# TingweiMeng/PDHG-optimal-control

Measured on AMD Instinct MI355X. Metric: PDHG iterations/sec and achieved HBM GB/s on nt×nx[×ny] grid, 1/2/4/8 MI355X, higher is better.
Workload: dtype f64

## Files before the change

include/pdhg.h:

```cpp
#ifndef PDHG_MI355X_H
#define PDHG_MI355X_H

#ifdef __cplusplus
extern "C" {
#endif

#define PDHG_ABI_VERSION 1

typedef enum pdhg_status {
  PDHG_OK = 0,
  PDHG_ERR_ARG = -1,
  PDHG_ERR_UNSUPPORTED = -2,
  PDHG_ERR_HIP = -3,
  PDHG_ERR_STATE = -4,
  PDHG_ERR_NOMEM = -5
} pdhg_status;

typedef struct pdhg_problem {
  int egno;
  int ndim;
  int bc_x, bc_y;
  int nx, ny;
  int T;
  int precision;
// ... 13 lines not shown
  int inner_last;
  int inner_total;
  double err1;
  double err2;
  double err_inner;
  double rho_min, rho_max;
  int nan_seen;
  int first_nan_iter;
} pdhg_stats;

typedef struct pdhg_ctx pdhg_ctx;

const char* pdhg_last_error(void);
int pdhg_abi_version(void);

int pdhg_device_count(int* count);

int pdhg_create(const pdhg_problem* prob, int device, pdhg_ctx** out);
int pdhg_destroy(pdhg_ctx* ctx);

int pdhg_set_state(pdhg_ctx* ctx, const double* phi, const double* rho, const double* alp);
int pdhg_get_state(pdhg_ctx* ctx, double* phi, double* rho, double* alp);
int pdhg_get_phi_bar(pdhg_ctx* ctx, double* phi_bar);
int pdhg_get_rows(pdhg_ctx* ctx, int row0, int nrows, double* phi, double* phi_bar, double* rho, double* alp);
int pdhg_set_phi_bar(pdhg_ctx* ctx, const double* phi_bar);

int pdhg_init_state(pdhg_ctx* ctx, const double* g);

int pdhg_update_primal(pdhg_ctx* ctx, double tau);

int pdhg_update_dual(pdhg_ctx* ctx, double sigma, double eps, int rho_alp_iters, int* inner_used);

int pdhg_errors(pdhg_ctx* ctx, double* err1, double* err2);

int pdhg_inner_error(pdhg_ctx* ctx, double* err);

int pdhg_iterate(pdhg_ctx* ctx, int n_iters, double tau, double sigma, double eps, int rho_alp_iters,
                 pdhg_stats* out);

int pdhg_set_stop_rules(pdhg_ctx* ctx, int stop_on_converge, int stop_on_nan);

int pdhg_synchronize(pdhg_ctx* ctx);

int pdhg_device_bytes(pdhg_ctx* ctx, unsigned long long* bytes);

int pdhg_path_info(pdhg_ctx* ctx, const char* key, int* value);
// ... 95 lines not shown
```

pdhg-optimal-control_amd/csrc/ctx_impl.hpp:

```cpp
#pragma once

#include <hip/hip_runtime.h>

#include <algorithm>
#include <climits>
#include <cmath>
#include <cstring>
#include <map>
#include <memory>
#include <string>
#include <type_traits>
#include <utility>
#include <vector>

#include "kernels_1d.hpp"
#include "kernels_2d.hpp"
#include "kernels_2d_fast.hpp"
#include "kernels_dual_lds.hpp"
#include "kernels_dual_multi.hpp"
#include "kernels_common.hpp"
#include "kernels_xslab.hpp"
#include "kernels_xt_batch.hpp"
#include "kernels_xt_dma.hpp"
#include "kernels_thomas_chunk.hpp"
// ... 609 lines not shown
          case 512: return launch(k_precond_x_t1_2d<512, 4, 512, double>, g, dim3(512), lds, p, twx);
          default: return fail(PDHG_ERR_UNSUPPORTED, "no fp64 one-row x kernel for nx=%d", p.nx);
        }
      }
      if (pp.f64_xt) {
        if (pp.half_real)
          return launch(k_precond_xt_f64_2d<4096, 512, true>, g, dim3(512),
                        (size_t)(Pad<4096>::LINE + TwLds<4096>::SIZE + 4096 + 128) * sizeof(C), p, twx);
        if (p.nx == 1024)
          return launch(k_precond_xt_f64_2d<1024, 256, false, true>, g, dim3(256),
                        (size_t)(Pad<1024>::LINE + TwLds<1024>::SIZE) * sizeof(C), p, twx);
        if (p.nx == 512)
          return launch(k_precond_xt_f64_2d<512, 128, false, true>, g, dim3(128),
                        (size_t)(Pad<512>::LINE + TwLds<512>::SIZE) * sizeof(C), p, twx);
        if (p.nx == 2048) {
          const size_t bpr = (size_t)(Pad<2048>::LINE + TwLds<2048>::SIZE) * sizeof(C);
          switch (pp.xt64_var) {
            case 1: return launch(k_precond_xt_f64_2d<2048, 256, false, false>, g, dim3(256), bpr + 2048 * sizeof(C), p, twx);
            case 2: return launch(k_precond_xt_f64_2d<2048, 256, false, true>, g, dim3(256), bpr, p, twx);
            case 3: return launch(k_precond_xt_f64_2d<2048, 1024, false, true>, g, dim3(1024), bpr, p, twx);
            default: return launch(k_precond_xt_f64_2d<2048, 512, false, true>, g, dim3(512), bpr, p, twx);
          }
        }
        const size_t lds = (size_t)(Pad<4096>::LINE + TwLds<4096>::SIZE + 4096) * sizeof(C);
        if (p.rspec)
          return launch(k_precond_xt_f64_2d<4096, 512, false, false, true>, g, dim3(512), lds, p, twx);
        return launch(k_precond_xt_f64_2d<4096, 512>, g, dim3(512), lds, p, twx);
      }
    }
    return with_xt_fft([&](auto f) {
      return launch(k_precond_xt_2d<R, decltype(f)>, g, dim3(pp.NT2), pp.lds_xt, p, f, twx);
    });
  }

  int launch_update_2d(const KP<R>& p, int& upd_rows) {
    ProfScope ps(this, "update");
    const dim3 gf(pp.g_fast_upd);
    upd_rows = pp.g_fast_upd;
    if constexpr (sizeof(R) == 8) {
      if (pp.res64) {
        if (pb.ny == 2048 && pp.upd_t1 > 0) {
          const size_t lds = pp.lds_res64 + (size_t)48 * sizeof(C);
          if (pp.upd_t1 == 2) return launch(k_invy_update_fast_2d<2048, 4, 256, 2, double, true>, gf, dim3(256), lds, p, twy);
          return launch(k_invy_update_fast_2d<2048, 4, 256, 4, double, true>, gf, dim3(256), lds, p, twy);
        }
        if (pb.ny == 4096) return launch(k_invy_update_fast_2d<4096, 4, 512, 4, double>, gf, dim3(512), pp.lds_upd64, p, twy);
// ... 816 lines not shown

  int set_phi_bar(const double* pbar) {
    const size_t n = (size_t)(pb.T + 1) * plane();
    if constexpr (sizeof(P) == 8) {
      H2D(phibar_dev(), pbar, n * sizeof(P));
      return PDHG_OK;
    }
    std::vector<R> buf(n);
    for (size_t i = 0; i < n; ++i) buf[i] = (R)pbar[i];
    H2D(kp.phibar, buf.data(), n * sizeof(R));
    return PDHG_OK;
  }

  int get_phi_bar(double* pbar) {
    HIP_TRY(hipStreamSynchronize(stream));
    const size_t n = (size_t)(pb.T + 1) * plane();
    if constexpr (kMixed) {
      HIP_TRY(hipMemcpy(pbar, px.phibar, n * sizeof(P), hipMemcpyDeviceToHost));
      return PDHG_OK;
    }
    std::vector<R> buf(n);
    HIP_TRY(hipMemcpy(buf.data(), kp.phibar, n * sizeof(R), hipMemcpyDeviceToHost));
    for (size_t i = 0; i < n; ++i) pbar[i] = (double)buf[i];
    return PDHG_OK;
  }

  int get_state(double* phi, double* rho, double* alp) {
    HIP_TRY(hipStreamSynchronize(stream));
    Ctrl h;
    int rc;
    if ((rc = read_ctrl(h))) return rc;
    const int cur = h.cur;
    const size_t npl = plane();
    const int T = pb.T;
    const size_t nphi = (size_t)(T + 1) * npl;
    std::unique_ptr<R[]> buf(new R[nphi]);
    const size_t n = (size_t)T * npl;
    auto plane_out = [&](double* dst, const auto* src, size_t cnt) -> int {
      using E = std::remove_cv_t<std::remove_pointer_t<decltype(src)>>;
      if constexpr (sizeof(E) == 8) {
        HIP_TRY(hipMemcpy(dst, src, cnt * sizeof(E), hipMemcpyDeviceToHost));
      } else {
        HIP_TRY(hipMemcpy(buf.get(), src, cnt * sizeof(E), hipMemcpyDeviceToHost));
        for (size_t i = 0; i < cnt; ++i) dst[i] = (double)buf[i];
      }
      return PDHG_OK;
// ... 368 lines not shown
```

pdhg-optimal-control_amd/csrc/fft_lds.hpp:

```cpp
#pragma once
#include "common.hpp"

namespace pdhg {

struct FFTPlan {
  int n;
  int npass;
  int pow2;
  int radix[kMaxPass];
};

__device__ constexpr double kC16[16] = {1.0, 0.92387953251128674, 0.70710678118654752, 0.38268343236508977,
                                        0.0, -0.38268343236508977, -0.70710678118654752, -0.92387953251128674,
                                        -1.0, -0.92387953251128674, -0.70710678118654752, -0.38268343236508977,
                                        0.0, 0.38268343236508977, 0.70710678118654752, 0.92387953251128674};
__device__ constexpr double kS16[16] = {0.0, 0.38268343236508977, 0.70710678118654752, 0.92387953251128674,
                                        1.0, 0.92387953251128674, 0.70710678118654752, 0.38268343236508977,
                                        0.0, -0.38268343236508977, -0.70710678118654752, -0.92387953251128674,
                                        -1.0, -0.92387953251128674, -0.70710678118654752, -0.38268343236508977};

template <typename C>
__device__ __forceinline__ void dft2(C& a, C& b) {
  const C t = a;
  a = cadd(t, b);
// ... 327 lines not shown
  lds_sync();
#pragma unroll
  for (int q = 0; q < PER; ++q) {
    if (base[q] >= 0) {
      dft_any<C, R>(v[q]);
      C* d = a + base[q];
#pragma unroll
      for (int r = 0; r < R; ++r) d[(LS == 1) ? r : r * (LS + LS / 16)] = v[q][r];
    }
  }
  lds_sync();
}

template <typename C, int N, int NL, int NT, int LS, bool REG, int LINE = Pad<N>::LINE, int GLS = (1 << 30)>
__device__ __forceinline__ void inplace_passes(C* a, const C* __restrict__ tw, const C* twl) {
  if constexpr (LS < N) {
    constexpr int rem = N / LS;
    constexpr int R = (rem >= 16) ? 16 : rem;
    inplace_pass<C, N, NL, NT, LS, R, REG, LINE, GLS>(a, tw, twl);
    inplace_passes<C, N, NL, NT, LS * R, REG, LINE, GLS>(a, tw, twl);
  }
}

template <typename C, int N, int NL, int NT, int LINE = Pad<N>::LINE>
__device__ __forceinline__ void lds_fft_inplace(C* a, const C* __restrict__ tw) {
  inplace_passes<C, N, NL, NT, 1, false, LINE>(a, tw, nullptr);
}

template <typename C, int N, int NL, int NT, int LINE = Pad<N>::LINE>
__device__ __forceinline__ void lds_fft_inplace_tl(C* a, const C* twl) {
  inplace_passes<C, N, NL, NT, 1, true, LINE>(a, nullptr, twl);
}

template <typename C, int N, int NL, int NT, int LINE = Pad<N>::LINE>
__device__ __forceinline__ void lds_fft_inplace_tl16(C* a, const C* twl, const C* __restrict__ tw) {
  inplace_passes<C, N, NL, NT, 1, true, LINE, 256>(a, tw, twl);
}


template <typename C, int N>
__device__ __forceinline__ void fill_twlds(C* twl, const C* __restrict__ tw, int tw_stride = 1,
                                           int cnt = TwLds<N>::SIZE) {
  for (int i = threadIdx.x; i < cnt; i += blockDim.x) {
    const int LS = i >= 816 ? 4096 : i >= 48 ? 256 : 16;
    const int e = i - twlds_off(LS);
    const int k = e / 3, m = e - 3 * k;
// ... 184 lines not shown
```

pdhg-optimal-control_amd/csrc/kernels_xt_f64.hpp:

```cpp
#pragma once
#include "kernels_2d_fast.hpp"

namespace pdhg {

__device__ __forceinline__ __amdgpu_buffer_rsrc_t row_rsrc(const double* base, int bytes) {
  return __builtin_amdgcn_make_buffer_rsrc(const_cast<double*>(base), 0, bytes, 0x00020000);
}
__device__ __forceinline__ double2 buf_ld2(__amdgpu_buffer_rsrc_t r, int voff, int soff) {
  return __builtin_bit_cast(double2, __builtin_amdgcn_raw_buffer_load_b128(r, voff, soff, 0));
}
__device__ __forceinline__ void buf_st2(__amdgpu_buffer_rsrc_t r, int voff, int soff, double2 v) {
  __builtin_amdgcn_raw_buffer_store_b128(__builtin_bit_cast(u32x4_t, v), r, voff, soff, 0);
}

__device__ __forceinline__ double eth_of(double dd) {
  return 1.0 / (1.0 + 0.5 * dd + sqrt(dd * (1.0 + 0.25 * dd)));
}
__device__ __forceinline__ double theta_of(double dd) {
  const double dl = 0.5 * dd;
  return fmax(log1p(dl + sqrt(dl * (dl + 2.0))), 1e-300);
}


template <int N, int NT, bool HR = false, bool BPR = false, bool TC = false>
__global__ void __launch_bounds__(NT) k_precond_xt_f64_2d(KP<double> p, const double2* __restrict__ twx) {
  using C = double2;
  constexpr int IT = N / NT;
  constexpr int LINE = Pad<N>::LINE;
  constexpr int M = 2 * N;
  static_assert(N % NT == 0 && N <= 4096 && IT <= 32, "one padded complex line and its twiddle seeds in LDS");
  if (p.ctrl->done) return;
  extern __shared__ __align__(16) unsigned char smem_raw[];
  C* A = reinterpret_cast<C*>(smem_raw);
  C* twl = A + LINE;
  C* bp = twl + TwLds<N>::SIZE;
  C* rsw = bp + (BPR ? 0 : N);
  static_assert(!(BPR && HR), "half-real blocks keep b' in LDS");
  static_assert(!TC || (!HR && !BPR && NT % 4 == 0), "task-order input: column pairs, 4-row tasks");
  fill_twlds<C, N>(twl, twx, HR ? 2 : 1);
  if constexpr (HR) {
    static_assert(N == 4096, "split-twiddle tables sized for 2N = 8192");
    for (int i = threadIdx.x; i < 128; i += blockDim.x) rsw[i] = twx[i < 64 ? i : 64 * (i - 64)];
  }
  const int T = p.T, tid = threadIdx.x;
  const int b = ((TC && !(p.dbg & 4096)) ? xcd_remap(blockIdx.x, gridDim.x) : (int)blockIdx.x) + p.b0;
  double* wb = p.work + (size_t)b * M;
  const size_t kstride = (size_t)p.nb * M;
  const double inv_ae = 1.0 / (double)p.ae;
  const double ly0 = p.lamy[HR ? b : 2 * b], ly1 = p.lamy[HR ? b : 2 * b + 1];
  auto kx_of = [&](int i) { return tid + i * NT; };
  auto dd_of = [&](int i) {
    const double lx0 = p.lamx[kx_of(i)], lx1 = HR ? (double)p.lamx[kx_of(i) + N] : lx0;
    return make_double2(((double)p.C - lx0 - ly0) * inv_ae, ((double)p.C - lx1 - ly1) * inv_ae);
  };
  auto unpack2 = [&](int i, double& h0, double& h1) {
    if constexpr (HR) {
      const int k = kx_of(i);
      realsplit_padded<C, double>(A, N, k, cmul(rsw[k & 63], rsw[64 + (k >> 6)]), h0, h1);
    } else {
      hartley_padded<C, double>(A, N, kx_of(i), h0, h1);
    }
  };
  auto stage2 = [&](int i, C x) {
    if constexpr (HR) {
      double* Af = reinterpret_cast<double*>(A);
      const int f0 = kx_of(i), f1 = kx_of(i) + N;
      Af[2 * pix(f0 >> 1) + (f0 & 1)] = x.x;
// ... 30 lines not shown
#pragma unroll
    for (int i = 0; i < IT; ++i) pf[i] = buf_ld2(r, voff, ioff(i));
  };
  const int ny_t = p.nb * 2;
  auto ldrow_in = [&](int kk) {
    if constexpr (TC) {
      const auto r = row_rsrc(p.rspec + (size_t)kk * kstride + (size_t)8 * b, (int)(kstride * sizeof(double)) - 64 * b);
      const int vin = 32 * ny_t * (tid >> 2) + 16 * (tid & 3);
#pragma unroll
      for (int i = 0; i < IT; ++i) pf[i] = buf_ld2(r, vin, 8 * ny_t * NT * i);
    } else {
      ldrow(kk);
    }
  };
  const int j0 = p.j0;
  const bool slab = p.slab != 0;
  if (p.xt_phase != 2) {
#pragma unroll
    for (int i = 0; i < IT; ++i) {
      c1[i] = dd_of(i);
      c2[i] = slab ? make_double2(h_entry(c1[i].x, j0), h_entry(c1[i].y, j0)) : make_double2(1.0, 1.0);
      bp_st(i, make_double2(0.0, 0.0));
    }
    ldrow_in(0);
    for (int k = 0; k < T; ++k) {
      const int kg = j0 + k;
      const bool nrow = k == T - 1 && p.last_slab;
#pragma unroll
      for (int i = 0; i < IT; ++i) A[pix(kx_of(i))] = pf[i];
      if (k + 1 < T) ldrow_in(k + 1);
      lds_sync();
      lds_fft_inplace_tl<C, N, 1, NT>(A, twl);
#pragma unroll
      for (int i = 0; i < IT; ++i)
        if (kg == max(kf[i], j0) && !nrow)
          c1[i] = make_double2(eth_of(c1[i].x), eth_of(c1[i].y));
      const auto dst = rowr(k);
#pragma unroll
      for (int i = 0; i < IT; ++i) {
        double ha, hb;
        unpack2(i, ha, hb);
        const C b0 = bp_ld(i);
        const double r0 = ha * inv_ae + b0.x, r1 = hb * inv_ae + b0.y;
        C bn;
        const int kfj = max(kf[i], j0);
        const bool fast = kg > kfj || (kg == kfj && !nrow);
        if (!nrow) {
          if (fast) {
            bn = make_double2(r0 * c1[i].x, r1 * c1[i].y);
          } else {
            const double s0 = c1[i].x + c2[i].x, s1 = c1[i].y + c2[i].y;
            const double g0 = 1.0 / (1.0 + s0), g1 = 1.0 / (1.0 + s1);
            bn = make_double2(r0 * g0, r1 * g1);
            c2[i] = make_double2(s0 * g0, s1 * g1);
          }
          buf_st2(dst, voff, ioff(i), bn);
        } else {
          if (fast) bn = make_double2(r0 * c1[i].x / (1.0 - c1[i].x), r1 * c1[i].y / (1.0 - c1[i].y));
          else bn = make_double2(r0 / (c1[i].x + c2[i].x), r1 / (c1[i].y + c2[i].y));
          if (slab) buf_st2(dst, voff, ioff(i), bn);
        }
        bp_st(i, bn);
      }
      lds_sync();
    }
  }
  if (p.xt_phase == 1) return;
  const int ks = slab ? T - 1 : T - 2;
#pragma unroll
  for (int i = 0; i < IT; ++i) {
    const C dd = dd_of(i);
    c1[i] = make_double2(theta_of(dd.x), theta_of(dd.y));
    if (j0 + ks >= kf[i]) {
      c2[i] = make_double2(exp(-c1[i].x), exp(-c1[i].y));
    } else {
      c2[i] = make_double2(expm1(-2.0 * c1[i].x * (j0 + ks + 2)), expm1(-2.0 * c1[i].y * (j0 + ks + 2)));
    }
    if (slab) bp_st(i, p.carry_y ? reinterpret_cast<const C*>(p.carry_y + (size_t)b * M)[kx_of(i)]
                                 : make_double2(0.0, 0.0));
  }
  if (ks >= 0) ldrow(ks);
  for (int k = T - 1; k >= 0; --k) {
    const int kg = j0 + k;
#pragma unroll
    for (int i = 0; i < IT; ++i)
      if (kg + 1 == kf[i] && k < ks)
        c2[i] = make_double2(expm1(-2.0 * c1[i].x * (kg + 2)), expm1(-2.0 * c1[i].y * (kg + 2)));
#pragma unroll
    for (int i = 0; i < IT; ++i) {
      C x = bp_ld(i);
      if (k <= ks) {
        double g0, g1;
        if (kg >= kf[i]) {
          g0 = c2[i].x;
          g1 = c2[i].y;
        } else {
          const double t0 = c1[i].x, t1 = c1[i].y;
          const double e0 = expm1(-2.0 * t0 * (kg + 1)), e1 = expm1(-2.0 * t1 * (kg + 1));
          g0 = t0 > 1e-150 ? exp(-t0) * e0 / c2[i].x : (double)(kg + 1) / (double)(kg + 2);
          g1 = t1 > 1e-150 ? exp(-t1) * e1 / c2[i].y : (double)(kg + 1) / (double)(kg + 2);
          c2[i] = make_double2(e0, e1);
        }
        x = make_double2(pf[i].x + g0 * x.x, pf[i].y + g1 * x.y);
        bp_st(i, x);
      }
      stage2(i, x);
// ... 22 lines not shown
```

pdhg-optimal-control_amd/csrc/path_plan.hpp:

```cpp
#pragma once

#include <cstdio>
#include <string>

#include "../../include/pdhg.h"
#include "fft_lds.hpp"
#include "kernels_dual_multi.hpp"
#include "kernels_fs16.hpp"
#include "tuning.hpp"

namespace pdhg {

constexpr size_t kLdsBytes = 160 * 1024;
constexpr int kMultiSub = 5;
constexpr int kMixedUpdPF = 4;
constexpr int kFoldRows = 64;

inline FFTPlan make_plan(int n, bool& ok) {
  FFTPlan pl{};
  pl.n = n;
  pl.pow2 = (n > 0) && ((n & (n - 1)) == 0);
  int m = n, np = 0;
  ok = true;
  auto push = [&](int r) {
// ... 50 lines not shown
  bool k1_outer = true;
  bool fold_fin = false;
  bool spec_ok = false;
  bool fin_merge = true;
  bool fuse_res = false;
  bool fast_rows = false;
  bool res64 = false;
  bool ip_rows = false;
  bool upd8192 = false;
  bool tc_spec = false;
  bool to_c4 = false;
  int res_threads = 0, upd_threads = 0;
  int res64_nt2048 = 512;
  int upd_t1 = 0;
  bool t1_xt = true;
  bool fast_xt = false;
  int fast_xt_code = 0;
  bool xt_dma = false, xt_pair = false;
  int xt_rpre = 0;
  bool t1_xt64 = false;
  bool t1_g16 = false;
  bool f64_xt = false;
  int xt64_var = 0;
  bool glb_line = false;
  bool fourstep = false;
  bool fs_wide = true;
  bool fs16 = false;
  int f16_group = 16;
  bool thomas_chunk = false;
  bool report_tile = false;
  int report_wgs = 1024;
};

inline int plan_paths(const pdhg_problem& pb, int S, const Decomp& dc, const Tuning& tn, PathPlan& pl,
                      std::string& err) {
  auto fail = [&err](int code, const char* fmt, auto... args) {
    if constexpr (sizeof...(args) == 0) {
      err = fmt;
    } else {
      char buf[512];
      snprintf(buf, sizeof(buf), fmt, args...);
      err = buf;
    }
    return code;
  };
  pl = PathPlan{};
// ... 8 lines not shown
  pl.n_dead = (pb.ndim == 2 && pb.egno == 3) ? 2 : 0;
  const bool two_sets = pl.two_sets = pb.rho_alp_iters > 1;
  bool ok1 = true, ok2 = true;
  pl.plx = make_plan(nxg, ok1);
  if (is2d) pl.ply = make_plan(ny, ok2);
  if (!ok1 || !ok2) return fail(PDHG_ERR_UNSUPPORTED, "FFT plan too deep for nx=%d ny=%d", nxg, ny);

  if (is2d) {
    const size_t cap = (S == 4) ? 8192 : 4096;
    int B = 16;
    while (B > 2 && (size_t)nxg * B > cap) B >>= 1;
    int nyp = 2;
    while (nyp < ny) nyp <<= 1;
    if (B > nyp) B = nyp;
    const bool xt64_on = tn.xt64.value_or(1) != 0;
    const bool f64_small = S == 8 && pb.bc_x == 0 && (slab ? dc.Tg : T) > 1 && (nxg == 1024 || nxg == 512) &&
                           ny % 2 == 0 && xt64_on;
    if (f64_small) B = 2;
    pl.half_real = nxg == 8192 && pb.bc_x == 0 && (S == 4 || !xslab);
    if (pl.half_real) B = 1;
    pl.f64_xt = S == 8 && pb.bc_x == 0 &&
                (((nxg == 4096 || nxg == 2048) && B == 2) || (nxg == 8192 && pl.half_real) || f64_small) && xt64_on;
    pl.xt64_var = tn.xt64_var;
    pl.t1_xt64 = S == 8 && T == 1 && pb.bc_x == 0 && !pl.half_real && !slab && pl.plx.pow2 &&
                 nxg >= 512 && nxg <= 4096 && nxg * (B / 2) == (nxg == 4096 ? 4096 : 2048);
    pl.res64_nt2048 = tn.res64_nt2048.value_or(T == 1 ? 256 : 512);
    pl.upd_t1 = T == 1 ? tn.upd_t1.value_or(2) : 0;
    if (!pl.half_real && !pl.f64_xt && (size_t)nxg * B > cap)
      return fail(PDHG_ERR_UNSUPPORTED, "nx=%d too large for the x-transform slab (max %zu in this precision)", nxg,
                  cap / 2);
    pl.B = B;
    while ((1 << pl.lB) < B) ++pl.lB;
    pl.nb = (ny + B - 1) / B;
    pl.lds_res = 2 * (size_t)ny * csz;
    const int nmodes = nxg * B;
    pl.lds_xt = (size_t)5 * nmodes * S;
    pl.ip_rows = S == 8 && ny == 8192 && pl.lds_res > kLdsBytes && !xslab;
    if (pl.ip_rows) pl.lds_res = (size_t)Pad<8192>::LINE * csz;
    pl.upd8192 = pl.ip_rows && pl.half_real && nx % 2 == 0 && tn.upd8192.value_or(1) != 0;
    if (pl.upd8192) pl.g_fast_upd = std::min((nx / 2) * T, 2048);
    if (pl.lds_res > kLdsBytes) return fail(PDHG_ERR_UNSUPPORTED, "ny=%d exceeds the LDS row transform", ny);
    {
      const int wg = (int)std::max<size_t>(1, kLdsBytes / std::max<size_t>(pl.lds_res, 1));
      pl.nt_row = std::min(1024, 256 * std::max(1, 4 / wg));
    }
    pl.NT2 = std::min(512, ((nmodes + 63) / 64) * 64);
// ... 166 lines not shown
  else if (k == "dual64") *value = (S == 8 && pl.fast_dual) ? 1 : 0;
  else if (k == "fast_dual") *value = pl.fast_dual ? pl.dual_rx : -1;
  else if (k == "dual_ypl") *value = pl.fast_dual && pl.dual_rx ? pl.dual_ypl : 0;
  else if (k == "res64_nt") *value = pl.res64 ? (pb.ny == 2048 ? pl.res64_nt2048 : 512) : 0;
  else if (k == "upd_t1") *value = (pl.res64 && pb.ny == 2048) ? pl.upd_t1 : 0;
  else if (k == "t1_g16") *value = (pl.t1_g16 && (pb.nx == 2048 || pb.nx == 4096)) ? 1 : 0;
  else if (k == "dual_one") *value = pl.dual_one ? 1 : 0;
  else if (k == "fast_xt") *value = pl.fast_xt_code;
  else if (k == "half_real") *value = pl.half_real ? 1 : 0;
  else if (k == "fourstep") *value = pl.fourstep ? 1 : 0;
  else if (k == "glb_line") *value = pl.glb_line ? 1 : 0;
  else if (k == "ip_rows") *value = pl.ip_rows ? 1 : 0;
  else if (k == "upd8192") *value = pl.upd8192 ? 1 : 0;
  else if (k == "tc_spec") *value = pl.tc_spec ? 1 : 0;
  else if (k == "to_c4") *value = pl.to_c4 ? 1 : 0;
  else if (k == "thomas_chunk") *value = pl.thomas_chunk ? 1 : 0;
  else if (k == "fs_wide") *value = (pl.fourstep && pl.fs_wide && !pl.fs16) ? 1 : 0;
  else if (k == "fs16") *value = pl.fs16 ? 1 : 0;
  else if (k == "rows_rw") *value = pl.fast_rows ? pl.RWf : 0;
  else if (k == "row_threads") *value = pl.nt_row;
  else if (k == "res_threads") *value = pl.res_threads;
  else if (k == "upd_threads") *value = pl.upd_threads;
  else if (k == "f64_xt") *value = pl.f64_xt ? 1 : 0;
  else if (k == "t1_xt64") *value = (pl.t1_xt64 && pl.t1_xt) ? 1 : 0;
  else if (k == "report_tile") *value = pl.report_tile ? 1 : 0;
  else if (k == "report_wgs") *value = pl.report_tile ? pl.report_wgs : 0;
  else return false;
  return true;
}

}
```

pdhg-optimal-control_amd/csrc/pdhg_api.hip:

```cpp
#include <hip/hip_runtime.h>

#include <cstdarg>
#include <cstdio>
#include <memory>
#include <string>

#include "../../include/pdhg.h"

namespace {

thread_local std::string g_err;

int fail(int code, const char* fmt, ...) {
  char buf[1024];
  va_list ap;
  va_start(ap, fmt);
  vsnprintf(buf, sizeof(buf), fmt, ap);
  va_end(ap);
  g_err = buf;
  return code;
}

#define HIP_TRY(expr)                                                                           \
  do {                                                                                          \
// ... 158 lines not shown
  if (rc) return rc;
  *out = reinterpret_cast<pdhg_ctx*>(box.release());
  return PDHG_OK;
}

int pdhg_destroy(pdhg_ctx* ctx) {
  if (!ctx) return PDHG_OK;
  CtxBox* b = ctx_box(ctx);
  if (!b) return fail(PDHG_ERR_ARG, "foreign context handle");
  b->magic = 0;
  delete b;
  return PDHG_OK;
}

int pdhg_set_state(pdhg_ctx* ctx, const double* phi, const double* rho, const double* alp) {
  return dispatch(ctx, [&](auto& im) { return im.set_state(phi, rho, alp); });
}
int pdhg_get_state(pdhg_ctx* ctx, double* phi, double* rho, double* alp) {
  return dispatch(ctx, [&](auto& im) { return im.get_state(phi, rho, alp); });
}
int pdhg_get_phi_bar(pdhg_ctx* ctx, double* phi_bar) {
  if (!phi_bar) return fail(PDHG_ERR_ARG, "null phi_bar");
  return dispatch(ctx, [&](auto& im) { return im.get_phi_bar(phi_bar); });
}
int pdhg_set_phi_bar(pdhg_ctx* ctx, const double* phi_bar) {
  if (!phi_bar) return fail(PDHG_ERR_ARG, "null phi_bar");
  return dispatch(ctx, [&](auto& im) { return im.set_phi_bar(phi_bar); });
}
int pdhg_get_rows(pdhg_ctx* ctx, int row0, int nrows, double* phi, double* phi_bar, double* rho, double* alp) {
  return dispatch(ctx, [&](auto& im) { return im.get_rows(row0, nrows, phi, phi_bar, rho, alp); });
}
int pdhg_init_state(pdhg_ctx* ctx, const double* g) {
  if (!g) return fail(PDHG_ERR_ARG, "null g");
  return dispatch(ctx, [&](auto& im) { return im.init_state(g); });
}
int pdhg_update_primal(pdhg_ctx* ctx, double tau) {
  return dispatch(ctx, [&](auto& im) { return im.update_primal(tau); });
}
int pdhg_update_dual(pdhg_ctx* ctx, double sigma, double eps, int rho_alp_iters, int* inner_used) {
  if (rho_alp_iters < 1) return fail(PDHG_ERR_ARG, "rho_alp_iters must be >= 1");
  return dispatch(ctx, [&](auto& im) { return im.update_dual(sigma, eps, rho_alp_iters, inner_used); });
}
int pdhg_errors(pdhg_ctx* ctx, double* err1, double* err2) {
  return dispatch(ctx, [&](auto& im) { return im.errors(err1, err2); });
}
int pdhg_inner_error(pdhg_ctx* ctx, double* err) {
// ... 373 lines not shown
```

pdhg-optimal-control_amd/csrc/tuning.hpp:

```cpp
#pragma once

#include <algorithm>
#include <cstdlib>
#include <cstring>
#include <optional>

namespace pdhg {

using EnvInt = std::optional<int>;

inline EnvInt env_int(const char* name) {
  const char* e = getenv(name);
  return e ? EnvInt(atoi(e)) : EnvInt();
}
inline int env_int(const char* name, int dflt) { return env_int(name).value_or(dflt); }
inline bool env_flag(const char* name, bool dflt) { return env_int(name, dflt ? 1 : 0) != 0; }

struct Tuning {
  int alloc_mode = 0;

  EnvInt xt64;
  int xt64_var = 0;
  bool t1_xt = true;
  bool t1_g16 = true;
  int short_t_xt = 16;
  EnvInt xt_ws;
  EnvInt xt_batch;
  int xt_rpre = 0;
  bool xt_pair = false;
  EnvInt xt_dma;
  EnvInt xt_dma_hr;

  EnvInt upd_t1;
  EnvInt res64_nt2048;
  EnvInt upd8192;
  int rows_var = 0;
  int half_nt = 3;
  int res64_nt = 512;
  int upd_pf = 4;
  EnvInt tile_j;
  EnvInt res64;
  EnvInt tc_spec;
  EnvInt fuse_res;
  EnvInt c4_to;

// ... 11 lines not shown
  EnvInt fs16;
  int f16_group = 16;
  EnvInt fuse_res1d;
  int fr1d_chunks = 8;
  EnvInt thomas_chunk;

  bool k1_outer = true;
  bool fold_fin = false;
  int g_outer = 2048;
  int head_xrun = 4;
  EnvInt dual_multi;
  EnvInt dual_head;
  EnvInt spec;
  bool fin_merge = true;

  EnvInt report_tile;
  int report_wgs = 1024;

  static Tuning from_env() {
    Tuning t;
    if (const char* e = getenv("PDHG_ALLOC")) t.alloc_mode = !strcmp(e, "contig") ? 1 : !strcmp(e, "none") ? -1 : 0;
    t.xt64 = env_int("PDHG_XT64");
    t.xt64_var = env_int("PDHG_XT64_VAR", t.xt64_var);
    t.t1_xt = env_flag("PDHG_T1_XT", t.t1_xt);
    t.t1_g16 = env_flag("PDHG_T1_G16", t.t1_g16);
    t.short_t_xt = env_int("PDHG_SHORT_T_XT", t.short_t_xt);
    t.xt_ws = env_int("PDHG_XT_WS");
    t.xt_batch = env_int("PDHG_XT_BATCH");
    t.xt_rpre = env_int("PDHG_XT_RPRE", t.xt_rpre);
    t.xt_pair = env_flag("PDHG_XT_PAIR", t.xt_pair);
    t.xt_dma = env_int("PDHG_XT_DMA");
    t.xt_dma_hr = env_int("PDHG_XT_DMA_HR");
    t.upd_t1 = env_int("PDHG_UPD_T1");
    if ((t.res64_nt2048 = env_int("PDHG_RES64_NT2048"))) t.res64_nt2048 = *t.res64_nt2048 == 256 ? 256 : 512;
    t.upd8192 = env_int("PDHG_UPD8192");
    t.rows_var = env_int("PDHG_ROWS_VAR", t.rows_var);
    t.half_nt = env_int("PDHG_HALF_NT", t.half_nt);
    t.res64_nt = env_int("PDHG_RES64_NT", t.res64_nt) == 1024 ? 1024 : 512;
    t.upd_pf = env_int("PDHG_UPD_PF", t.upd_pf);
    t.tile_j = env_int("PDHG_TILE_J");
    t.res64 = env_int("PDHG_RES64");
    t.tc_spec = env_int("PDHG_TC_SPEC");
    t.fuse_res = env_int("PDHG_FUSE_RES");
    t.c4_to = env_int("PDHG_C4_TO");
    t.short_t_dual = env_int("PDHG_SHORT_T", t.short_t_dual);
    t.dual64 = env_int("PDHG_DUAL64");
// ... 62 lines not shown
```

pdhg-optimal-control_amd/pdhg_amd/_native.py:

```python
import ctypes
import os

import numpy as np

_HERE = os.path.dirname(os.path.abspath(__file__))
LIB_PATH = os.path.join(_HERE, "libpdhg.so")

PDHG_OK = 0
PDHG_ERR_ARG = -1
PDHG_ERR_UNSUPPORTED = -2
PDHG_ERR_HIP = -3
PDHG_ERR_STATE = -4
PDHG_ERR_NOMEM = -5

EXPORTS = (
    "pdhg_last_error", "pdhg_abi_version", "pdhg_device_count", "pdhg_create", "pdhg_destroy",
    "pdhg_set_state", "pdhg_get_state", "pdhg_get_phi_bar", "pdhg_set_phi_bar", "pdhg_get_rows", "pdhg_init_state",
    "pdhg_update_primal", "pdhg_update_dual", "pdhg_errors", "pdhg_inner_error", "pdhg_iterate", "pdhg_set_stop_rules", "pdhg_synchronize",
    "pdhg_device_bytes", "pdhg_path_info", "pdhg_plan_info", "pdhg_profile_enable", "pdhg_profile_query", "pdhg_algorithmic_bytes",
    "pdhg_trajectories",
    "pdhg_report_state", "pdhg_report_rows",
    "pdhg_create_slab", "pdhg_set_stream", "pdhg_slab_plane_size", "pdhg_slab_begin", "pdhg_slab_carry_gain",
    "pdhg_slab_residual", "pdhg_slab_forward", "pdhg_slab_fixup", "pdhg_slab_long_modes", "pdhg_slab_fixup_nb", "pdhg_slab_backward", "pdhg_slab_primal_finalize", "pdhg_slab_dual",
    "pdhg_slab_dual_finalize", "pdhg_slab_outer", "pdhg_slab_outer_finalize", "pdhg_slab_plane_out",
    "pdhg_slab_plane_in", "pdhg_slab_status", "pdhg_slab_part_modes", "pdhg_slab_forward_part",
    "pdhg_slab_carry_out_part", "pdhg_slab_fixup_nb_part", "pdhg_slab_backward_part", "pdhg_slab_update",
    "pdhg_create_xslab", "pdhg_xslab_layout", "pdhg_xslab_sizes", "pdhg_xslab_halo_out", "pdhg_xslab_halo_in",
    "pdhg_xslab_residual", "pdhg_xslab_wire", "pdhg_xslab_precond", "pdhg_xslab_update",
    "pdhg_create_multi", "pdhg_multi_destroy", "pdhg_multi_set_state", "pdhg_multi_get_state",
    "pdhg_multi_iterate", "pdhg_multi_set_stop_rules", "pdhg_multi_synchronize", "pdhg_multi_info",
    "pdhg_multi_profile", "pdhg_multi_phase_ms", "pdhg_multi_init_state", "pdhg_build_id",
)


class PDHGError(RuntimeError):
    def __init__(self, code, msg):
        super().__init__("pdhg status {}: {}".format(code, msg))
        self.code = code


# ... 51 lines not shown

def load():
    global _lib
    if _lib is not None:
        return _lib
    if not os.path.exists(LIB_PATH):
        raise ImportError("libpdhg.so not built at {} — run __graft_entry__.build()".format(LIB_PATH))
    try:
        import torch
    except ImportError:
        pass
    lib = ctypes.CDLL(LIB_PATH)
    P = ctypes.c_void_p
    dp = ctypes.POINTER(ctypes.c_double)
    sig = {
        "pdhg_last_error": ([], ctypes.c_char_p),
        "pdhg_abi_version": ([], ctypes.c_int),
        "pdhg_device_count": ([ctypes.POINTER(ctypes.c_int)], ctypes.c_int),
        "pdhg_create": ([ctypes.POINTER(pdhg_problem), ctypes.c_int, ctypes.POINTER(P)], ctypes.c_int),
        "pdhg_destroy": ([P], ctypes.c_int),
        "pdhg_set_state": ([P, dp, dp, dp], ctypes.c_int),
        "pdhg_get_state": ([P, dp, dp, dp], ctypes.c_int),
        "pdhg_get_phi_bar": ([P, dp], ctypes.c_int),
        "pdhg_set_phi_bar": ([P, dp], ctypes.c_int),
        "pdhg_get_rows": ([P, ctypes.c_int, ctypes.c_int, dp, dp, dp, dp], ctypes.c_int),
        "pdhg_init_state": ([P, dp], ctypes.c_int),
        "pdhg_update_primal": ([P, ctypes.c_double], ctypes.c_int),
        "pdhg_update_dual": ([P, ctypes.c_double, ctypes.c_double, ctypes.c_int, ctypes.POINTER(ctypes.c_int)],
                             ctypes.c_int),
        "pdhg_errors": ([P, dp, dp], ctypes.c_int),
        "pdhg_inner_error": ([P, dp], ctypes.c_int),
        "pdhg_iterate": ([P, ctypes.c_int, ctypes.c_double, ctypes.c_double, ctypes.c_double, ctypes.c_int,
                          ctypes.POINTER(pdhg_stats)], ctypes.c_int),
        "pdhg_set_stop_rules": ([P, ctypes.c_int, ctypes.c_int], ctypes.c_int),
        "pdhg_synchronize": ([P], ctypes.c_int),
        "pdhg_device_bytes": ([P, ctypes.POINTER(ctypes.c_ulonglong)], ctypes.c_int),
        "pdhg_path_info": ([P, ctypes.c_char_p, ctypes.POINTER(ctypes.c_int)], ctypes.c_int),
        "pdhg_plan_info": ([ctypes.POINTER(pdhg_problem), ctypes.c_char_p, ctypes.POINTER(ctypes.c_int)], ctypes.c_int),
        "pdhg_profile_enable": ([P, ctypes.c_int], ctypes.c_int),
        "pdhg_profile_query": ([P, ctypes.c_char_p, dp, ctypes.POINTER(ctypes.c_int)], ctypes.c_int),
        "pdhg_algorithmic_bytes": ([P, ctypes.c_int, ctypes.c_char_p, dp], ctypes.c_int),
        "pdhg_trajectories": ([P, ctypes.POINTER(pdhg_traj_opts), dp, dp, dp, dp, dp], ctypes.c_int),
        "pdhg_report_state": ([P, ctypes.POINTER(pdhg_report)], ctypes.c_int),
        "pdhg_report_rows": ([P, ctypes.c_int, ctypes.c_int, dp, dp], ctypes.c_int),
        "pdhg_create_slab": ([ctypes.POINTER(pdhg_problem), ctypes.c_int, ctypes.c_int, ctypes.c_int,
                              ctypes.POINTER(P)], ctypes.c_int),
# ... 84 lines not shown
```

pdhg-optimal-control_amd/pdhg_amd/context.py:

```python
import ctypes

import numpy as np

from . import _native as N


def traj_arguments(ndim, T, x_init, method, x_period, y_period=None, center=(False, False), noise=None,
                   record=("x", "alp"), seed=0, sample_offset=0):
    if method not in N.TRAJ_METHODS:
        raise ValueError("method must be 'linear' or 'nearest', not {!r}".format(method))
    record = (record,) if isinstance(record, str) else tuple(record or ())
    if set(record) - {"x", "alp"}:
        raise ValueError("record takes 'x' and / or 'alp', not {!r}".format(record))
    x0 = np.ascontiguousarray(x_init, dtype=np.float64)
    want = "[n_sample]" if ndim == 1 else "[n_sample, 2]"
    if x0.ndim != ndim or (ndim == 2 and x0.shape[1] != 2) or x0.shape[0] < 1:
        raise ValueError("x_init must be {} with n_sample >= 1, not {}".format(want, x0.shape))
    n = x0.shape[0]
    if ndim == 2 and y_period is None:
        raise ValueError("y_period is required in 2-D")
    if not (x_period > 0) or (ndim == 2 and not (y_period > 0)):
        raise ValueError("periods must be > 0")
    if len(tuple(center)) != 2:
        raise ValueError("center is a pair (center_x, center_y)")
# ... 94 lines not shown
                len(alp) == len(r[2]) and all(a is b for a, b in zip(alp, r[2])))

    def get_state(self, phi=True, rho=True, alp=True):
        phi = np.empty((self.T + 1,) + self._space) if phi else None
        rho = np.empty((self.T,) + self._space) if rho else None
        alp = np.empty((self.n_alp, self.T) + self._space + (self.n_ctrl,)) if alp else None
        N.check(self._lib.pdhg_get_state(self._h, N.dptr(phi), N.dptr(rho), N.dptr(alp)))
        return phi, rho, (None if alp is None else tuple(alp[i] for i in range(self.n_alp)))

    def get_rows(self, row0, nrows, phi=True, phi_bar=False, rho=True, alp=True):
        sp = self._space
        f = lambda on: np.empty((nrows,) + sp) if on else None
        a = np.empty((self.n_alp, nrows) + sp + (self.n_ctrl,)) if alp else None
        ph, pb, rh = f(phi), f(phi_bar), f(rho)
        N.check(self._lib.pdhg_get_rows(self._h, int(row0), int(nrows), N.dptr(ph), N.dptr(pb), N.dptr(rh),
                                        N.dptr(a)))
        return ph, pb, rh, (None if a is None else tuple(a[i] for i in range(self.n_alp)))

    def get_phi_bar(self):
        pb = np.empty((self.T + 1,) + self._space)
        N.check(self._lib.pdhg_get_phi_bar(self._h, N.dptr(pb)))
        return pb

    def set_phi_bar(self, phi_bar):
        self._version += 1
        pb = np.ascontiguousarray(phi_bar, dtype=np.float64).reshape((self.T + 1,) + self._space)
        N.check(self._lib.pdhg_set_phi_bar(self._h, N.dptr(pb)))

    def init_state(self, g):
        g = np.ascontiguousarray(g, dtype=np.float64).reshape(self._space)
        self._version += 1
        N.check(self._lib.pdhg_init_state(self._h, N.dptr(g)))

    def trajectories(self, x_init, method, x_period, y_period=None, center=(False, False), noise=None, seed=0,
                     record=("x", "alp"), sample_offset=0):
        o, x0, noise, rec_x, rec_a = traj_arguments(self.ndim, self.T, x_init, method, x_period, y_period, center,
                                                    noise, record, seed, sample_offset)
        n = x0.shape[0]
        tail = () if self.ndim == 1 else (2,)
        x_final = np.empty((n,) + tail)
        traj_x = np.empty((self.T + 1, n) + tail) if rec_x else None
        traj_alp = np.empty((self.T, n, self.n_ctrl)) if rec_a else None
        N.check(self._lib.pdhg_trajectories(self._h, ctypes.byref(o), N.dptr(x0), N.dptr(noise), N.dptr(x_final),
                                            N.dptr(traj_x), N.dptr(traj_alp)))
        return traj_alp, traj_x, x_final

# ... 69 lines not shown
```

Baseline: 8.520.

## Stage f64 xt preconditioner rows into LDS with async global-load-to-LDS DMA

For the nx=4096, column-pair f64 xt preconditioner path, adds a DMA variant that prefetches the next time row straight into an LDS staging buffer with global_load_lds. The first FFT pass then reads out-of-place from that buffer with hand-written ds_read_b128 batches, and the b' stores are moved after the FFT with a counted vmcnt wait. It also enables the b'-in-registers (BPR) variant by default for this configuration. The aim is to overlap the HBM row loads with the LDS FFT and free registers, at the cost of more static LDS, inline asm fragility and fixed waitcnt encodings. A debug accessor for the work buffer is added as well.

```diff
diff --git a/include/pdhg.h b/include/pdhg.h
--- a/include/pdhg.h
+++ b/include/pdhg.h
@@ -59,6 +59,7 @@
 int pdhg_set_state(pdhg_ctx* ctx, const double* phi, const double* rho, const double* alp);
 int pdhg_get_state(pdhg_ctx* ctx, double* phi, double* rho, double* alp);
 int pdhg_get_phi_bar(pdhg_ctx* ctx, double* phi_bar);
+int pdhg_get_work(pdhg_ctx* ctx, double* out, long long count);
 int pdhg_get_rows(pdhg_ctx* ctx, int row0, int nrows, double* phi, double* phi_bar, double* rho, double* alp);
 int pdhg_set_phi_bar(pdhg_ctx* ctx, const double* phi_bar);
 
diff --git a/pdhg-optimal-control_amd/csrc/ctx_impl.hpp b/pdhg-optimal-control_amd/csrc/ctx_impl.hpp
--- a/pdhg-optimal-control_amd/csrc/ctx_impl.hpp
+++ b/pdhg-optimal-control_amd/csrc/ctx_impl.hpp
@@ -655,6 +655,15 @@
             default: return launch(k_precond_xt_f64_2d<2048, 512, false, true>, g, dim3(512), bpr, p, twx);
           }
         }
+        if (pp.xt64_dma) {
+          if (p.rspec) return launch(k_precond_xt_f64_2d<4096, 512, false, true, true, true>, g, dim3(512), 0, p, twx);
+          return launch(k_precond_xt_f64_2d<4096, 512, false, true, false, true>, g, dim3(512), 0, p, twx);
+        }
+        if (pp.xt64_bpr) {
+          const size_t ldsr = (size_t)(Pad<4096>::LINE + TwLds<4096>::SIZE) * sizeof(C);
+          if (p.rspec) return launch(k_precond_xt_f64_2d<4096, 512, false, true, true>, g, dim3(512), ldsr, p, twx);
+          return launch(k_precond_xt_f64_2d<4096, 512, false, true>, g, dim3(512), ldsr, p, twx);
+        }
         const size_t lds = (size_t)(Pad<4096>::LINE + TwLds<4096>::SIZE + 4096) * sizeof(C);
         if (p.rspec)
           return launch(k_precond_xt_f64_2d<4096, 512, false, false, true>, g, dim3(512), lds, p, twx);
@@ -1517,6 +1526,16 @@
     std::vector<R> buf(n);
     HIP_TRY(hipMemcpy(buf.data(), kp.phibar, n * sizeof(R), hipMemcpyDeviceToHost));
     for (size_t i = 0; i < n; ++i) pbar[i] = (double)buf[i];
+    return PDHG_OK;
+  }
+
+  int get_work(double* out, size_t count) {
+    HIP_TRY(hipStreamSynchronize(stream));
+    const size_t nwork = pb.ndim == 2 ? (size_t)pb.T * kp.nb * pb.nx * kp.B : (size_t)pb.T * pb.nx;
+    if (count > nwork) return fail(PDHG_ERR_ARG, "work buffer holds %zu elements", nwork);
+    std::vector<R> buf(count);
+    HIP_TRY(hipMemcpy(buf.data(), kp.work, count * sizeof(R), hipMemcpyDeviceToHost));
+    for (size_t i = 0; i < count; ++i) out[i] = (double)buf[i];
     return PDHG_OK;
   }
 
diff --git a/pdhg-optimal-control_amd/csrc/fft_lds.hpp b/pdhg-optimal-control_amd/csrc/fft_lds.hpp
--- a/pdhg-optimal-control_amd/csrc/fft_lds.hpp
+++ b/pdhg-optimal-control_amd/csrc/fft_lds.hpp
@@ -373,6 +373,26 @@
   }
 }
 
+template <typename C, int N, int NT, class RD>
+__device__ __forceinline__ void first_pass_oop(C* __restrict__ a, RD&& read16) {
+  constexpr int nR = N / 16;
+  static_assert(nR % 16 == 0 && nR <= NT, "padded schedule, one butterfly per thread");
+  const int j = threadIdx.x;
+  C v[16];
+  int base = -1;
+  if (j < nR) {
+    read16(j, v);
+    base = pix(j * 16);
+  }
+  asm volatile("" : "+v"(base)::"memory");
+  if (base >= 0) {
+    dft_any<C, 16>(v);
+    C* d = a + base;
+#pragma unroll
+    for (int r = 0; r < 16; ++r) d[r] = v[r];
+  }
+}
+
 template <typename C, int N, int NL, int NT, int LINE = Pad<N>::LINE>
 __device__ __forceinline__ void lds_fft_inplace(C* a, const C* __restrict__ tw) {
   inplace_passes<C, N, NL, NT, 1, false, LINE>(a, tw, nullptr);
diff --git a/pdhg-optimal-control_amd/csrc/kernels_xt_f64.hpp b/pdhg-optimal-control_amd/csrc/kernels_xt_f64.hpp
--- a/pdhg-optimal-control_amd/csrc/kernels_xt_f64.hpp
+++ b/pdhg-optimal-control_amd/csrc/kernels_xt_f64.hpp
@@ -1,5 +1,6 @@
 #pragma once
 #include "kernels_2d_fast.hpp"
+#include "kernels_xt_dma.hpp"
 
 namespace pdhg {
 
@@ -11,6 +12,24 @@
 }
 __device__ __forceinline__ void buf_st2(__amdgpu_buffer_rsrc_t r, int voff, int soff, double2 v) {
   __builtin_amdgcn_raw_buffer_store_b128(__builtin_bit_cast(u32x4_t, v), r, voff, soff, 0);
+}
+
+__device__ __forceinline__ void s_read16(unsigned a, double2 (&v)[16]) {
+  typedef double d2v __attribute__((ext_vector_type(2)));
+  d2v w[16];
+  asm volatile(
+      "ds_read_b128 %0, %16\n\tds_read_b128 %1, %16 offset:4096\n\tds_read_b128 %2, %16 offset:8192\n\t"
+      "ds_read_b128 %3, %16 offset:12288\n\tds_read_b128 %4, %16 offset:16384\n\tds_read_b128 %5, %16 offset:20480\n\t"
+      "ds_read_b128 %6, %16 offset:24576\n\tds_read_b128 %7, %16 offset:28672\n\tds_read_b128 %8, %16 offset:32768\n\t"
+      "ds_read_b128 %9, %16 offset:36864\n\tds_read_b128 %10, %16 offset:40960\n\tds_read_b128 %11, %16 offset:45056\n\t"
+      "ds_read_b128 %12, %16 offset:49152\n\tds_read_b128 %13, %16 offset:53248\n\t"
+      "ds_read_b128 %14, %16 offset:57344\n\tds_read_b128 %15, %16 offset:61440\n\ts_waitcnt lgkmcnt(0)"
+      : "=&v"(w[0]), "=&v"(w[1]), "=&v"(w[2]), "=&v"(w[3]), "=&v"(w[4]), "=&v"(w[5]), "=&v"(w[6]), "=&v"(w[7]),
+        "=&v"(w[8]), "=&v"(w[9]), "=&v"(w[10]), "=&v"(w[11]), "=&v"(w[12]), "=&v"(w[13]), "=&v"(w[14]), "=&v"(w[15])
+      : "v"(a)
+      : "memory");
+#pragma unroll
+  for (int r = 0; r < 16; ++r) v[r] = make_double2(w[r].x, w[r].y);
 }
 
 __device__ __forceinline__ double eth_of(double dd) {
@@ -22,27 +41,39 @@
 }
 
 
-template <int N, int NT, bool HR = false, bool BPR = false, bool TC = false>
+template <int N, int NT, bool HR = false, bool BPR = false, bool TC = false, bool DMA = false>
 __global__ void __launch_bounds__(NT) k_precond_xt_f64_2d(KP<double> p, const double2* __restrict__ twx) {
   using C = double2;
   constexpr int IT = N / NT;
   constexpr int LINE = Pad<N>::LINE;
   constexpr int M = 2 * N;
   static_assert(N % NT == 0 && N <= 4096 && IT <= 32, "one padded complex line and its twiddle seeds in LDS");
+  static_assert(!DMA || (BPR && !HR && N == 4096 && NT == 512), "DMA staging: the nx = 4096 column-pair form");
   if (p.ctrl->done) return;
   extern __shared__ __align__(16) unsigned char smem_raw[];
-  C* A = reinterpret_cast<C*>(smem_raw);
-  C* twl = A + LINE;
+  C *A, *twl, *S = nullptr;
+  if constexpr (DMA) {
+    __shared__ __align__(16) C A_s[LINE];
+    __shared__ __align__(16) C S_s[N];
+    __shared__ __align__(16) C twl_s[TwLds<N>::SIZE];
+    A = A_s;
+    S = S_s;
+    twl = twl_s;
+  } else {
+    A = reinterpret_cast<C*>(smem_raw);
+    twl = A + LINE;
+  }
   C* bp = twl + TwLds<N>::SIZE;
   C* rsw = bp + (BPR ? 0 : N);
   static_assert(!(BPR && HR), "half-real blocks keep b' in LDS");
-  static_assert(!TC || (!HR && !BPR && NT % 4 == 0), "task-order input: column pairs, 4-row tasks");
+  static_assert(!TC || (!HR && NT % 4 == 0), "task-order input: column pairs, 4-row tasks");
   fill_twlds<C, N>(twl, twx, HR ? 2 : 1);
   if constexpr (HR) {
     static_assert(N == 4096, "split-twiddle tables sized for 2N = 8192");
     for (int i = threadIdx.x; i < 128; i += blockDim.x) rsw[i] = twx[i < 64 ? i : 64 * (i - 64)];
   }
-  const int T = p.T, tid = threadIdx.x;
+  const int T = p.T;
+  int tid = threadIdx.x;
   const int b = ((TC && !(p.dbg & 4096)) ? xcd_remap(blockIdx.x, gridDim.x) : (int)blockIdx.x) + p.b0;
   double* wb = p.work + (size_t)b * M;
   const size_t kstride = (size_t)p.nb * M;
@@ -119,15 +150,40 @@
       c2[i] = slab ? make_double2(h_entry(c1[i].x, j0), h_entry(c1[i].y, j0)) : make_double2(1.0, 1.0);
       bp_st(i, make_double2(0.0, 0.0));
     }
-    ldrow_in(0);
+    const int wave = __builtin_amdgcn_readfirstlane(tid >> 6);
+    auto issue_row = [&](auto kk) {
+      const char* src = TC ? reinterpret_cast<const char*>(p.rspec + (size_t)kk * kstride + (size_t)8 * b) +
+                                 (32 * ny_t * (tid >> 2) + 16 * (tid & 3))
+                           : reinterpret_cast<const char*>(wb + (size_t)kk * kstride) + voff;
+#pragma unroll
+      for (int i = 0; i < IT; ++i)
+        __builtin_amdgcn_global_load_lds(
+            reinterpret_cast<const u32x4_t*>(src + (TC ? (size_t)8 * ny_t * NT * i : (size_t)ioff(i))),
+            (__attribute__((address_space(3))) void*)(S + i * NT + wave * 64), 16, 0, 0);
+    };
+    if constexpr (DMA) {
+      issue_row(0);
+      __builtin_amdgcn_s_waitcnt(0x0F70);
+      lds_sync();
+    } else {
+      ldrow_in(0);
+    }
     for (int k = 0; k < T; ++k) {
       const int kg = j0 + k;
       const bool nrow = k == T - 1 && p.last_slab;
-#pragma unroll
-      for (int i = 0; i < IT; ++i) A[pix(kx_of(i))] = pf[i];
-      if (k + 1 < T) ldrow_in(k + 1);
-      lds_sync();
-      lds_fft_inplace_tl<C, N, 1, NT>(A, twl);
+      if constexpr (DMA) {
+        if (!(p.dbg & 8192))
+          first_pass_oop<C, N, NT>(A, [&](int j, C(&v)[16]) { s_read16(lds_addr(S + j), v); });
+        lds_sync();
+        if (k + 1 < T) issue_row(k + 1);
+        inplace_passes<C, N, 1, NT, 16, true>(A, nullptr, twl);
+      } else {
+#pragma unroll
+        for (int i = 0; i < IT; ++i) A[pix(kx_of(i))] = pf[i];
+        if (k + 1 < T) ldrow_in(k + 1);
+        lds_sync();
+        lds_fft_inplace_tl<C, N, 1, NT>(A, twl);
+      }
 #pragma unroll
       for (int i = 0; i < IT; ++i)
         if (kg == max(kf[i], j0) && !nrow)
@@ -151,13 +207,27 @@
             bn = make_double2(r0 * g0, r1 * g1);
             c2[i] = make_double2(s0 * g0, s1 * g1);
           }
-          buf_st2(dst, voff, ioff(i), bn);
+          if constexpr (!DMA) buf_st2(dst, voff, ioff(i), bn);
         } else {
           if (fast) bn = make_double2(r0 * c1[i].x / (1.0 - c1[i].x), r1 * c1[i].y / (1.0 - c1[i].y));
           else bn = make_double2(r0 / (c1[i].x + c2[i].x), r1 / (c1[i].y + c2[i].y));
-          if (slab) buf_st2(dst, voff, ioff(i), bn);
+          if constexpr (!DMA) if (slab) buf_st2(dst, voff, ioff(i), bn);
         }
         bp_st(i, bn);
+      }
+      if constexpr (DMA) {
+        static_assert(IT == 8, "the counted wait below is vmcnt(8)");
+        if (k + 1 < T) {
+#pragma unroll
+          for (int i = 0; i < IT; ++i) buf_st2(dst, voff, ioff(i), bpr[i]);
+          __builtin_amdgcn_s_waitcnt(0x0F78);
+        } else {
+          if (!nrow || slab) {
+#pragma unroll
+            for (int i = 0; i < IT; ++i) buf_st2(dst, voff, ioff(i), bpr[i]);
+          }
+          __builtin_amdgcn_s_waitcnt(0x0F70);
+        }
       }
       lds_sync();
     }
@@ -179,6 +249,7 @@
   if (ks >= 0) ldrow(ks);
   for (int k = T - 1; k >= 0; --k) {
     const int kg = j0 + k;
+    if constexpr (BPR && IT == 8) asm volatile("" : "+v"(tid));
 #pragma unroll
     for (int i = 0; i < IT; ++i)
       if (kg + 1 == kf[i] && k < ks)
diff --git a/pdhg-optimal-control_amd/csrc/path_plan.hpp b/pdhg-optimal-control_amd/csrc/path_plan.hpp
--- a/pdhg-optimal-control_amd/csrc/path_plan.hpp
+++ b/pdhg-optimal-control_amd/csrc/path_plan.hpp
@@ -96,6 +96,8 @@
   bool t1_g16 = false;
   bool f64_xt = false;
   int xt64_var = 0;
+  bool xt64_bpr = false;
+  bool xt64_dma = false;
   bool glb_line = false;
   bool fourstep = false;
   bool fs_wide = true;
@@ -150,6 +152,12 @@
     pl.f64_xt = S == 8 && pb.bc_x == 0 &&
                 (((nxg == 4096 || nxg == 2048) && B == 2) || (nxg == 8192 && pl.half_real) || f64_small) && xt64_on;
     pl.xt64_var = tn.xt64_var;
+    {
+      const bool ok = pl.f64_xt && nxg == 4096 && B == 2 && !pl.half_real && !slab && !xslab;
+      const bool dma = ok && tn.xt64_dma.value_or(1) != 0;
+      pl.xt64_bpr = ok && tn.xt64_bpr.value_or(dma ? 1 : 0) != 0;
+      pl.xt64_dma = dma && pl.xt64_bpr;
+    }
     pl.t1_xt64 = S == 8 && T == 1 && pb.bc_x == 0 && !pl.half_real && !slab && pl.plx.pow2 &&
                  nxg >= 512 && nxg <= 4096 && nxg * (B / 2) == (nxg == 4096 ? 4096 : 2048);
     pl.res64_nt2048 = tn.res64_nt2048.value_or(T == 1 ? 256 : 512);
@@ -362,6 +370,8 @@
   else if (k == "res_threads") *value = pl.res_threads;
   else if (k == "upd_threads") *value = pl.upd_threads;
   else if (k == "f64_xt") *value = pl.f64_xt ? 1 : 0;
+  else if (k == "xt64_dma") *value = pl.xt64_dma ? 1 : 0;
+  else if (k == "xt64_bpr") *value = pl.xt64_bpr ? 1 : 0;
   else if (k == "t1_xt64") *value = (pl.t1_xt64 && pl.t1_xt) ? 1 : 0;
   else if (k == "report_tile") *value = pl.report_tile ? 1 : 0;
   else if (k == "report_wgs") *value = pl.report_tile ? pl.report_wgs : 0;
diff --git a/pdhg-optimal-control_amd/csrc/pdhg_api.hip b/pdhg-optimal-control_amd/csrc/pdhg_api.hip
--- a/pdhg-optimal-control_amd/csrc/pdhg_api.hip
+++ b/pdhg-optimal-control_amd/csrc/pdhg_api.hip
@@ -204,6 +204,10 @@
 int pdhg_get_phi_bar(pdhg_ctx* ctx, double* phi_bar) {
   if (!phi_bar) return fail(PDHG_ERR_ARG, "null phi_bar");
   return dispatch(ctx, [&](auto& im) { return im.get_phi_bar(phi_bar); });
+}
+int pdhg_get_work(pdhg_ctx* ctx, double* out, long long count) {
+  if (!out) return fail(PDHG_ERR_ARG, "null out");
+  return dispatch(ctx, [&](auto& im) { return im.get_work(out, count < 0 ? 0 : (size_t)count); });
 }
 int pdhg_set_phi_bar(pdhg_ctx* ctx, const double* phi_bar) {
   if (!phi_bar) return fail(PDHG_ERR_ARG, "null phi_bar");
diff --git a/pdhg-optimal-control_amd/csrc/tuning.hpp b/pdhg-optimal-control_amd/csrc/tuning.hpp
--- a/pdhg-optimal-control_amd/csrc/tuning.hpp
+++ b/pdhg-optimal-control_amd/csrc/tuning.hpp
@@ -21,6 +21,8 @@
 
   EnvInt xt64;
   int xt64_var = 0;
+  EnvInt xt64_dma;
+  EnvInt xt64_bpr;
   bool t1_xt = true;
   bool t1_g16 = true;
   int short_t_xt = 16;
@@ -78,6 +80,8 @@
     if (const char* e = getenv("PDHG_ALLOC")) t.alloc_mode = !strcmp(e, "contig") ? 1 : !strcmp(e, "none") ? -1 : 0;
     t.xt64 = env_int("PDHG_XT64");
     t.xt64_var = env_int("PDHG_XT64_VAR", t.xt64_var);
+    t.xt64_dma = env_int("PDHG_XT64_DMA");
+    t.xt64_bpr = env_int("PDHG_XT64_BPR");
     t.t1_xt = env_flag("PDHG_T1_XT", t.t1_xt);
     t.t1_g16 = env_flag("PDHG_T1_G16", t.t1_g16);
     t.short_t_xt = env_int("PDHG_SHORT_T_XT", t.short_t_xt);
diff --git a/pdhg-optimal-control_amd/pdhg_amd/_native.py b/pdhg-optimal-control_amd/pdhg_amd/_native.py
--- a/pdhg-optimal-control_amd/pdhg_amd/_native.py
+++ b/pdhg-optimal-control_amd/pdhg_amd/_native.py
@@ -15,7 +15,7 @@
 
 EXPORTS = (
     "pdhg_last_error", "pdhg_abi_version", "pdhg_device_count", "pdhg_create", "pdhg_destroy",
-    "pdhg_set_state", "pdhg_get_state", "pdhg_get_phi_bar", "pdhg_set_phi_bar", "pdhg_get_rows", "pdhg_init_state",
+    "pdhg_set_state", "pdhg_get_state", "pdhg_get_phi_bar", "pdhg_get_work", "pdhg_set_phi_bar", "pdhg_get_rows", "pdhg_init_state",
     "pdhg_update_primal", "pdhg_update_dual", "pdhg_errors", "pdhg_inner_error", "pdhg_iterate", "pdhg_set_stop_rules", "pdhg_synchronize",
     "pdhg_device_bytes", "pdhg_path_info", "pdhg_plan_info", "pdhg_profile_enable", "pdhg_profile_query", "pdhg_algorithmic_bytes",
     "pdhg_trajectories",
@@ -113,6 +113,7 @@
         "pdhg_set_state": ([P, dp, dp, dp], ctypes.c_int),
         "pdhg_get_state": ([P, dp, dp, dp], ctypes.c_int),
         "pdhg_get_phi_bar": ([P, dp], ctypes.c_int),
+        "pdhg_get_work": ([P, dp, ctypes.c_longlong], ctypes.c_int),
         "pdhg_set_phi_bar": ([P, dp], ctypes.c_int),
         "pdhg_get_rows": ([P, ctypes.c_int, ctypes.c_int, dp, dp, dp, dp], ctypes.c_int),
         "pdhg_init_state": ([P, dp], ctypes.c_int),
diff --git a/pdhg-optimal-control_amd/pdhg_amd/context.py b/pdhg-optimal-control_amd/pdhg_amd/context.py
--- a/pdhg-optimal-control_amd/pdhg_amd/context.py
+++ b/pdhg-optimal-control_amd/pdhg_amd/context.py
@@ -140,6 +140,11 @@
         N.check(self._lib.pdhg_get_phi_bar(self._h, N.dptr(pb)))
         return pb
 
+    def get_work(self, count):
+        out = np.empty(int(count))
+        N.check(self._lib.pdhg_get_work(self._h, N.dptr(out), int(count)))
+        return out
+
     def set_phi_bar(self, phi_bar):
         self._version += 1
         pb = np.ascontiguousarray(phi_bar, dtype=np.float64).reshape((self.T + 1,) + self._space)
```

New measurement: 8.694, median of 6. +2.0%, better.
